# shiinamiyuki/akari_render

Measured on AMD Instinct MI355X. Metric: Msamples/s (whole node), 1080p path tracer, C2, higher is better.
Workload: dtype f32

## Files before the change

akari_render_amd/capi.py:

```python
from __future__ import annotations

import ctypes as C
import os
from typing import Optional

import numpy as np

from . import abi
from .build import LIB, build

AKR_OK = 0
FILM_PLANE_RGB, FILM_PLANE_SPLAT, FILM_PLANE_WEIGHT, FILM_PLANES_PT, FILM_PLANES_ALL = 1, 2, 4, 5, 7
ERR_INVALID_ARGUMENT, ERR_HIP, ERR_NO_DEVICE, ERR_IO, ERR_PARSE, ERR_UNSUPPORTED, ERR_OOM, ERR_RENDER = -1, -2, -3, -4, -5, -6, -7, -8

(ARRAY_WOOP, ARRAY_TRI_GID, ARRAY_SHADE, ARRAY_INSTANCES, ARRAY_MATERIALS, ARRAY_BVH_NODES, ARRAY_LIGHT_ENTRIES,
 ARRAY_LIGHT_PDF, ARRAY_AREA_ENTRIES, ARRAY_AREA_PDF, ARRAY_INST_TRI_OFFSET, ARRAY_R2C, ARRAY_C2W,
 ARRAY_TEX_NODES, ARRAY_TEX_IMAGES, ARRAY_TEX_TEXELS, ARRAY_MAT_INPUTS,
 ARRAY_INST_LEAVES, ARRAY_MESH_TRIS, ARRAY_MESH_POS, ARRAY_MESH_META, ARRAY_MESH_NORMALS,
 ARRAY_ENV_MARGINAL_ENTRIES, ARRAY_ENV_MARGINAL_PDF, ARRAY_ENV_CONDITIONAL_ENTRIES, ARRAY_ENV_CONDITIONAL_PDF, ARRAY_ENV_TEXELS) = range(27)
ENV_LIGHT_INSTANCE = 0xFFFFFFFF

EXPORTS = [
    "akr_last_error", "akr_version", "akr_struct_size", "akr_option_set", "akr_option_get", "akr_context_create",
    "akr_context_destroy", "akr_context_synchronize", "akr_context_device_info", "akr_scene_create", "akr_scene_load",
# ... 6 lines not shown
    "akr_gpt_config_default", "akr_gpt_render", "akr_gpt_begin", "akr_gpt_sample", "akr_gpt_sums", "akr_gpt_sums_read",
    "akr_gpt_sums_write", "akr_gpt_finish", "akr_gpt_abort", "akr_gpt_reduce", "akr_mcmc_config_default", "akr_mcmc_render",
    "akr_film_set_splat_scale", "akr_film_get_splat_scale", "akr_pt_read_sampler_states", "akr_context_device_ordinal",
    "akr_device_count", "akr_comm_unique_id", "akr_comm_create", "akr_comm_wrap", "akr_comm_destroy", "akr_film_reduce",
    "akr_pt_kernel_info", "akr_scene_spec_source", "akr_host_spec_compile", "akr_host_spec_compile_text",
    "akr_film_reduce_planes", "akr_mcmc_render_shard", "akr_mcmc_combine_host", "akr_mcmc_combine",
    "akr_scene_set_environment", "akr_scene_get_environment", "akr_scene_set_lens", "akr_scene_get_lens",
]
TEST_EXPORTS = [
    "akr_probe_material_inputs_host", "akr_host_stdrng_u64", "akr_host_chacha_block", "akr_host_pcg32_states",
    "akr_host_pcg_start", "akr_host_alias_table", "akr_probe_math", "akr_probe_bsdf", "akr_probe_intersect",
    "akr_probe_surface_interaction", "akr_probe_material_inputs", "akr_host_decode_png", "akr_host_decode_jpeg",
    "akr_host_decode_exr", "akr_host_decode_tiff", "akr_host_decode_dds", "akr_host_pmj02bn_tables",
    "akr_probe_material_folded_host", "akr_host_sobol_dim1", "akr_host_fastmod", "akr_host_tri_pretest",
    "akr_probe_env_sample", "akr_probe_env_pdf", "akr_host_lens_ray", "akr_probe_camera_rays",
]


class RenderSession(C.Structure):

    _fields_ = [("save_intermediate", C.c_int32), ("save_stats", C.c_int32), ("name", C.c_char_p),
                ("override_sampler_independent", C.c_int32), ("verbose", C.c_int32)]


class AkariError(RuntimeError):
    def __init__(self, code: int, msg: str):
        super().__init__(f"akari_hip error {code}: {msg}")
        self.code = code


# ... 105 lines not shown
    proto("akr_pt_begin", vp, vp, C.POINTER(abi.PtConfig), vp, vpp)
    proto("akr_pt_passes", vp, u32, i32, up)
    proto("akr_pt_end", vp, C.POINTER(abi.PtStats))
    proto("akr_pt_get_stats", vp, C.POINTER(abi.PtStats))
    proto("akr_render_task", vp, vp, C.c_char_p, C.POINTER(RenderSession), C.POINTER(abi.PtStats))
    proto("akr_image_write", C.c_char_p, fp, u32, u32)
    proto("akr_pt_read_sampler_states", vp, u64p)
    proto("akr_host_stdrng_u64", u64, u32, u64p)
    proto("akr_host_chacha_block", up, u64, u64, i32, up)
    proto("akr_host_pcg32_states", u64, u64, u64p)
    proto("akr_host_pcg_start", u64p, u64)
    proto("akr_host_alias_table", fp, u32, up, fp, fp)
    proto("akr_probe_math", vp, u32, fp, fp, fp, fp)
    proto("akr_probe_bsdf", vp, C.POINTER(abi.MaterialDesc), fp, i32, fp, u32, fp, fp)
    proto("akr_probe_intersect", vp, vp, u32, fp, up, fp)
    proto("akr_probe_surface_interaction", vp, vp, u32, up, fp, fp)
    proto("akr_probe_material_inputs", vp, vp, u32, u32, fp, fp)
    proto("akr_probe_material_inputs_host", vp, u32, u32, u32, fp, fp)
    proto("akr_host_decode_png", C.c_char_p, u64, up, up, C.POINTER(C.c_uint8), u64)
    proto("akr_host_decode_jpeg", C.c_char_p, u64, up, up, C.POINTER(C.c_uint8), u64)
    proto("akr_host_decode_exr", C.c_char_p, u64, up, up, fp, u64)
    proto("akr_host_decode_tiff", C.c_char_p, u64, up, up, C.POINTER(C.c_uint8), u64)
    proto("akr_host_decode_dds", C.c_char_p, u64, up, up, C.POINTER(C.c_uint8), u64)
    proto("akr_host_pmj02bn_tables", up, C.POINTER(C.c_uint16))
    _lib = L
    return L


def check(rc: int) -> None:
    if rc != AKR_OK:
# ... 482 lines not shown
    w = np.ascontiguousarray(weights, dtype=np.float32)
    j = np.zeros(w.size, dtype=np.uint32)
    t = np.zeros(w.size, dtype=np.float32)
    pdf = np.zeros(w.size, dtype=np.float32)
    check(lib().akr_host_alias_table(_fp(w), w.size, _up(j), _fp(t), _fp(pdf)))
    return j, t, pdf


def probe_math(ctx: Context, x: np.ndarray):
    x = np.ascontiguousarray(x, dtype=np.float32)
    s, c, l = (np.zeros_like(x) for _ in range(3))
    check(lib().akr_probe_math(ctx.h, x.size, _fp(x), _fp(s), _fp(c), _fp(l)))
    return s, c, l


def probe_bsdf(ctx: Context, m: abi.MaterialData, mode: int, wo, data: np.ndarray, table: Optional[np.ndarray] = None) -> np.ndarray:
    ms = m.to_struct()
    wo = np.ascontiguousarray(wo, dtype=np.float32)
    data = np.ascontiguousarray(data, dtype=np.float32).reshape(-1, 3)
    out = np.zeros((data.shape[0], 4 if mode == 0 else 8), dtype=np.float32)
    tp = _fp(np.ascontiguousarray(table, dtype=np.float32)) if table is not None else C.POINTER(C.c_float)()
    check(lib().akr_probe_bsdf(ctx.h, C.byref(ms), tp, mode, _fp(wo), data.shape[0], _fp(data), _fp(out)))
    return out


def probe_intersect(ctx: Context, scene: Scene, rays: np.ndarray):
    rays = np.ascontiguousarray(rays, dtype=np.float32).reshape(-1, 8)
    out = np.zeros((rays.shape[0], 3), dtype=np.uint32)
    bary = np.zeros((rays.shape[0], 2), dtype=np.float32)
    check(lib().akr_probe_intersect(ctx.h, scene.h, rays.shape[0], _fp(rays), _up(out), _fp(bary)))
    return out, bary


def probe_surface_interaction(ctx: Context, scene: Scene, inst_prim: np.ndarray, bary: np.ndarray) -> np.ndarray:
    ip = np.ascontiguousarray(inst_prim, dtype=np.uint32).reshape(-1, 2)
    b = np.ascontiguousarray(bary, dtype=np.float32).reshape(-1, 2)
    out = np.zeros((ip.shape[0], 19), dtype=np.float32)
    check(lib().akr_probe_surface_interaction(ctx.h, scene.h, ip.shape[0], _up(ip), _fp(b), _fp(out)))
    return out


def probe_material_inputs(ctx: Optional[Context], scene: Scene, material: int, uv: np.ndarray) -> np.ndarray:
    u = np.ascontiguousarray(uv, dtype=np.float32).reshape(-1, 2)
    out = np.zeros((u.shape[0], 26), dtype=np.float32)
    check(lib().akr_probe_material_inputs(ctx.h if ctx is not None else C.c_void_p(), scene.h, material, u.shape[0], _fp(u), _fp(out)))
    return out
# ... 142 lines not shown
```

akari_render_amd/csrc/device/disect.h:

```cpp
#pragma once
#include "drng.h"
#include "dscene.h"

namespace akr {

template <bool V>
struct BoolTag {
    static constexpr bool value = V;
};

struct Hit {
    float t, u, v;
    uint32_t gid;
};

struct PlaneHit {
    float t, px, py, pz;
};
AKR_HD PlaneHit tri_plane(vec3 o, vec3 d, float4 r2) {
    float dz = __builtin_fmaf(r2.x, d.x, __builtin_fmaf(r2.y, d.y, r2.z * d.z));
    float oz = __builtin_fmaf(r2.x, o.x, __builtin_fmaf(r2.y, o.y, __builtin_fmaf(r2.z, o.z, r2.w)));
    PlaneHit h;
    h.t = div_f(-oz, dz);
    h.px = __builtin_fmaf(h.t, d.x, o.x);
// ... 95 lines not shown
    return best != kInvalid;
}

typedef float v2f __attribute__((ext_vector_type(2)));
typedef float v4f __attribute__((ext_vector_type(4)));
AKR_D float min_raw(float a, float b) {
    float r;
    asm("v_min_f32 %0, %1, %2" : "=v"(r) : "v"(a), "v"(b));
    return r;
}
AKR_D float max_raw(float a, float b) {
    float r;
    asm("v_max_f32 %0, %1, %2" : "=v"(r) : "v"(a), "v"(b));
    return r;
}
template <bool TEX = false>
AKR_D void trace_pair_exhaustive(const DScene& sc, vec3 o, vec3 d, float tmax, uint32_t ex0, vec3 so, vec3 sd, float stmax,
                                 uint32_t sex0, uint32_t sex1, Hit& hit, bool& found, bool& occluded, const float4* lds_recs) {
    float best_t = next_up(tmax);
    uint32_t best = kInvalid;
    float best_u = 0.0f, best_v = 0.0f;
    float occ_margin = -1.0f;
    const uint32_t n = sc.n_tris;
    const v4f* lrec = (const v4f*)lds_recs;
    const bool has_alpha = __builtin_amdgcn_readfirstlane((int)sc.has_alpha) != 0;
    v2f T2 = {0.0f, 0.0f}, hx2 = {0.0f, 0.0f}, hy2 = {0.0f, 0.0f}, hz2 = {0.0f, 0.0f};
    auto record = [&](auto alpha_tag, uint32_t k, const v4f& q0, const v4f& q1, const v4f& q2) {
        constexpr bool ALPHA = decltype(alpha_tag)::value;
        if (!((sc.plane_share_mask >> k) & 1ull)) {
            const PlaneHit a = tri_plane(o, d, make_float4(q2.x, q2.y, q2.z, q2.w)), b = tri_plane(so, sd, make_float4(q2.x, q2.y, q2.z, q2.w));
            T2 = (v2f){a.t, b.t};
            hx2 = (v2f){a.px, b.px}; hy2 = (v2f){a.py, b.py}; hz2 = (v2f){a.pz, b.pz};
        }
        float u, v, su, sv;
        tri_uv(PlaneHit{T2.x, hx2.x, hy2.x, hz2.x}, make_float4(q0.x, q0.y, q0.z, q0.w), make_float4(q1.x, q1.y, q1.z, q1.w), u, v);
        tri_uv(PlaneHit{T2.y, hx2.y, hy2.y, hz2.y}, make_float4(q0.x, q0.y, q0.z, q0.w), make_float4(q1.x, q1.y, q1.z, q1.w), su, sv);
        const v2f u2 = {u, su}, v2 = {v, sv};
        const v2f s2 = {1.0f - (u2.x + v2.x), 1.0f - (u2.y + v2.y)};
        const v2f w2 = {tmax - T2.x, stmax - T2.y};
        float m = min_raw(min_raw(min_raw(u2.x, v2.x), s2.x), min_raw(T2.x, w2.x));
        float sm = min_raw(min_raw(min_raw(u2.y, v2.y), s2.y), min_raw(T2.y, w2.y));
        m = (k == ex0) ? -1.0f : m;
        sm = (k == sex0) ? -1.0f : sm;
        sm = (k == sex1) ? -1.0f : sm;
        if (ALPHA) {
            const uint32_t ka = __builtin_amdgcn_readfirstlane(k);
            if (m >= 0.0f && !alpha_test<TEX>(sc, ka, u2.x, v2.x)) m = -1.0f;
            if (sm >= 0.0f && !alpha_test<TEX>(sc, ka, u2.y, v2.y)) sm = -1.0f;
        }
        const float tc = (m >= 0.0f) ? T2.x : __builtin_inff();
        const bool better = tc < best_t;
        best_t = better ? tc : best_t;
        best = better ? k : best;
        occ_margin = max_raw(occ_margin, sm);
    };
    auto walk = [&](auto alpha_tag) {
        v4f a0 = lrec[0], a1 = lrec[1], a2 = lrec[2], b0, b1, b2;
        uint32_t k = 0;
        for (; k + 1 < n; k += 2) {
            b0 = lrec[3 * (k + 1)]; b1 = lrec[3 * (k + 1) + 1]; b2 = lrec[3 * (k + 1) + 2];
            record(alpha_tag, k, a0, a1, a2);
            a0 = lrec[3 * (k + 2)]; a1 = lrec[3 * (k + 2) + 1]; a2 = lrec[3 * (k + 2) + 2];
            record(alpha_tag, k + 1, b0, b1, b2);
        }
        if (k < n) record(alpha_tag, k, a0, a1, a2);
    };
    if (has_alpha) walk(BoolTag<true>{});
    else walk(BoolTag<false>{});
    if (best != kInvalid) {
        const v4f q0 = lrec[3 * best], q1 = lrec[3 * best + 1];
        const float px = __builtin_fmaf(best_t, d.x, o.x), py = __builtin_fmaf(best_t, d.y, o.y), pz = __builtin_fmaf(best_t, d.z, o.z);
        best_u = __builtin_fmaf(q0.x, px, __builtin_fmaf(q0.y, py, __builtin_fmaf(q0.z, pz, q0.w)));
        best_v = __builtin_fmaf(q1.x, px, __builtin_fmaf(q1.y, py, __builtin_fmaf(q1.z, pz, q1.w)));
    }
    found = best != kInvalid;
    hit.t = found ? best_t : tmax;
    hit.u = best_u;
    hit.v = best_v;
    hit.gid = best;
    occluded = occ_margin >= 0.0f;
}

constexpr uint32_t kBvhDone = 0xfffffffeu;
// ... 235 lines not shown
```

akari_render_amd/csrc/device/dmath.h:

```cpp
#pragma once
#if !defined(__HIPCC_RTC__)
#include <hip/hip_runtime.h>
#include <stdint.h>
#else
typedef unsigned char uint8_t;
typedef unsigned short uint16_t;
typedef int int32_t;
typedef unsigned int uint32_t;
typedef long int64_t;
typedef unsigned long uint64_t;
typedef unsigned long uintptr_t;
typedef unsigned long size_t;
#endif

#define AKR_HD __host__ __device__ __forceinline__
#define AKR_D __device__ __forceinline__

#ifndef AKR_ARITH_RELAXED
#define AKR_ARITH_RELAXED 0
#endif
#if AKR_ARITH_RELAXED && defined(__HIP_DEVICE_COMPILE__)
#define AKR_RX 1
#else
#define AKR_RX 0
// ... 27 lines not shown
AKR_HD vec3 operator-(vec3 a) { return vec3{-a.x, -a.y, -a.z}; }
AKR_HD float dot(vec3 a, vec3 b) { return (a.x * b.x + a.y * b.y) + a.z * b.z; }
AKR_HD vec3 cross(vec3 a, vec3 b) { return vec3{a.y * b.z - a.z * b.y, a.z * b.x - a.x * b.z, a.x * b.y - a.y * b.x}; }
AKR_HD float rcp_f(float x) {
#if AKR_RX && AKR_RX_RCP
    return __builtin_amdgcn_rcpf(x);
#else
    return 1.0f / x;
#endif
}
AKR_HD float div_f(float a, float b) {
#if AKR_RX && AKR_RX_RCP
    return a * __builtin_amdgcn_rcpf(b);
#else
    return a / b;
#endif
}
AKR_HD float sqrt_f(float x) {
#if AKR_RX
    return __builtin_amdgcn_sqrtf(x);
#else
    return __builtin_sqrtf(x);
#endif
}
AKR_HD float length2(vec3 a) { return dot(a, a); }
AKR_HD float length(vec3 a) { return sqrt_f(dot(a, a)); }
AKR_HD vec3 div_s(vec3 a, float s) {
    float inv = rcp_f(s);
    return a * inv;
}
// ... 123 lines not shown
```

akari_render_amd/csrc/device/dscene.h:

```cpp
#pragma once
#include "dtex.h"

namespace akr {

constexpr uint32_t kInvalid = 0xffffffffu;

constexpr uint32_t kBvhNodeWords = 16;
constexpr uint32_t kBvhTriWords = 16;
constexpr uint32_t kBvhStackDepth = 24;

enum : uint32_t { SHADE_ROWS = 8, INST_ROWS = 8 };
enum : uint32_t { TRI_HAS_NORMALS = 1u, TRI_HAS_TANGENTS = 2u };

struct LightRec {
    uint32_t tri_offset, n_tris, first_gid, inst;
};

constexpr uint32_t kMeshPrimMask = 0x7fffffffu, kMeshTriShares = 0x80000000u;
struct DInst {
    const uint4* __restrict__ tlas_leaves;
    const float4* __restrict__ mesh_tris;
    const uint32_t* __restrict__ mesh_pos;
    const uint32_t* __restrict__ mesh_meta;
    const float4* __restrict__ mesh_normals;
// ... 107 lines not shown
```

akari_render_amd/csrc/device/pt_pass.h:

```cpp
#pragma once
#include "dpath.h"

namespace akr {

#ifndef AKR_PT_MIN_WAVES
#define AKR_PT_MIN_WAVES 4
#endif
#ifndef AKR_PT_MIN_WAVES_BVH
#define AKR_PT_MIN_WAVES_BVH 4
#endif
#ifndef AKR_PT_MIN_WAVES_FD
#define AKR_PT_MIN_WAVES_FD 4
#endif
#ifndef AKR_PT_MIN_WAVES_TEX
#define AKR_PT_MIN_WAVES_TEX 3
#endif
#ifndef AKR_PT_MIN_WAVES_BVH_TEX
#define AKR_PT_MIN_WAVES_BVH_TEX 3
#endif
template <bool BVH, bool FD, bool TEX, bool PMJ, bool STAGE, bool DEFER, uint32_t ABSENT = 0, bool INST = false, bool ENV = false, bool LENS = false>
AKR_D void pt_pass_body(const PtParams& p) {
    extern __shared__ __attribute__((aligned(16))) uint32_t lds_stack[];
    TraceCtx tc;
    tc.stack = lds_stack + threadIdx.x;
    tc.cnt = TraceCounters{0, 0, 0};
    PtParams staged = p;
    if (STAGE) stage_scene_tables<BVH, TEX, !BVH && !FD && TEX>(p, lds_stack, staged);
    const PtParams& q = STAGE ? staged : p;
    const DScene& sc = q.sc;
    constexpr bool TILE = BVH && !TEX && !INST;
    constexpr uint32_t STRAG = BVH ? (INST ? AKR_PT_STRAGGLERS_INST : (TEX ? AKR_PT_STRAGGLERS_TEX : AKR_PT_STRAGGLERS)) : 0;
    const uint4* tile = (const uint4*)(lds_stack + p.tile_offset);
    if (TILE) {
        uint32_t* l = lds_stack + p.tile_offset;
// ... 97 lines not shown
                while (phase != 2u) {
                    if (s.active) trav_step<2, TEX, TILE>(sc, s, tc.stack, tc.cnt, phase == 1u, tile);
                    if (!s.active) {
                        if (phase == 0u) {
                            found = s.best != kInvalid;
                            hit.t = s.best_t; hit.u = s.best_u; hit.v = s.best_v; hit.gid = s.best;
                            phase = r.has_shadow ? 1u : 2u;
                            if (r.has_shadow) trav_begin(s, r.s_o, r.s_d, 0.0f, r.s_tmax, r.s_ex0, r.s_ex1);
                        } else {
                            occluded = s.best != kInvalid;
                            phase = 2u;
                        }
                    }
                }
            } else {
                trace_pair_exhaustive<TEX>(sc, r.ro, r.rd, r.has_ray ? 1e20f : -1.0f, r.ray_ex0, r.s_o, r.s_d, r.has_shadow ? r.s_tmax : -1.0f, r.s_ex0, r.s_ex1, hit, found,
                                           occluded, lds_recs);
            }
            if (DEFER) {
                if (r.deferred) {
                    hit.gid = r.d_gid; hit.u = r.d_u; hit.v = r.d_v; hit.t = 0.0f;
                    found = true;
                    r.has_ray = true;
                    r.deferred = false;
                } else if (r.has_ray && found && (iteration & q.defer_metal)) {
                    const uint32_t mat = f2u(sc.shade[(size_t)hit.gid * SHADE_ROWS + 6].y);
                    if (sc.materials[mat].flags & q.defer_flags) {
                        r.d_gid = hit.gid; r.d_u = hit.u; r.d_v = hit.v;
                        r.deferred = true;
                        r.has_ray = false;
                    }
// ... 16 lines not shown
```

akari_render_amd/csrc/host/api_probe.cpp:

```cpp
#if defined(AKR_TEST_HOOKS) && AKR_TEST_HOOKS
#include "api_internal.h"
#include "../../../include/akari_hip_test.h"
#include "../device/dinst.h"
#include "../device/disect.h"
#include "../device/dpath.h"

extern "C" {

AKR_TEST_API int32_t akr_host_stdrng_u64(uint64_t seed, uint32_t n, uint64_t* out) {
    if (!out) return fail(AKR_ERR_INVALID_ARGUMENT, "out is NULL");
    StdRng rng(seed);
    for (uint32_t i = 0; i < n; i++) out[i] = rng.next_u64();
    return AKR_OK;
}
AKR_TEST_API int32_t akr_host_chacha_block(const uint32_t* key8, uint64_t counter, uint64_t stream, int32_t rounds, uint32_t* out16) {
    if (!key8 || !out16) return fail(AKR_ERR_INVALID_ARGUMENT, "NULL argument");
    StdRng::chacha_block(key8, counter, stream, rounds, out16);
    return AKR_OK;
}
AKR_TEST_API int32_t akr_host_pcg32_states(uint64_t seed, uint64_t n, uint64_t* out2n) {
    if (!out2n) return fail(AKR_ERR_INVALID_ARGUMENT, "out is NULL");
    StdRng rng(seed);
    for (uint64_t i = 0; i < n; i++) {
        Pcg32 p = pcg_new_seq_offset(i, rng.next_u64());
// ... 54 lines not shown
    return guarded([&] {
        ctx->bind();
        DevBuf dx, ds, dc, dl;
        std::vector<float> xv(x, x + n);
        dx.upload(xv);
        ds.alloc(n * 4); dc.alloc(n * 4); dl.alloc(n * 4);
        if (n) HIP_CHECK(launch_probe_math(n, dx.as<float>(), ds.as<float>(), dc.as<float>(), dl.as<float>(), ctx->stream));
        HIP_CHECK(hipStreamSynchronize(ctx->stream));
        if (n) {
            HIP_CHECK(hipMemcpy(s, ds.p, n * 4, hipMemcpyDeviceToHost));
            HIP_CHECK(hipMemcpy(c, dc.p, n * 4, hipMemcpyDeviceToHost));
            HIP_CHECK(hipMemcpy(l, dl.p, n * 4, hipMemcpyDeviceToHost));
        }
    });
}
AKR_TEST_API int32_t akr_probe_bsdf(akr_context* ctx, const akr_material_desc* m, const float* table, int32_t mode, const float* wo, uint32_t n,
                               const float* in, float* out) {
    if (!ctx || !m || !wo || !in || !out) return fail(AKR_ERR_INVALID_ARGUMENT, "akr_probe_bsdf: NULL argument");
    return guarded([&] {
        ctx->bind();
        std::vector<DMaterial> dm(1, fold_material(*m));
        DevBuf dmat, dtab, din, dout;
        dmat.upload(dm);
        std::vector<float> tab(4096, 0.0f);
        if (table) tab.assign(table, table + 4096);
        dtab.upload(tab);
        std::vector<float> inv(in, in + 3ull * n);
        din.upload(inv);
        size_t out_n = (mode == 0 ? 4ull : 8ull) * n;
        dout.alloc(out_n * 4);
// ... 11 lines not shown
}
AKR_TEST_API int32_t akr_probe_intersect(akr_context* ctx, akr_scene* scene, uint32_t n, const float* rays, uint32_t* hit_inst_prim, float* bary) {
    if (!ctx || !scene || !rays || !hit_inst_prim || !bary) return fail(AKR_ERR_INVALID_ARGUMENT, "akr_probe_intersect: NULL argument");
    return guarded([&] {
        ctx->bind();
        DevBuf dr, dout, db;
        std::vector<float> rv(rays, rays + 8ull * n);
        dr.upload(rv);
        dout.alloc(3ull * n * 4);
        db.alloc(2ull * n * 4);
        if (n) HIP_CHECK(launch_probe_intersect(probe_params(scene), n, dr.as<float>(), dout.as<uint32_t>(), db.as<float>(), ctx->stream));
        HIP_CHECK(hipStreamSynchronize(ctx->stream));
        if (n) {
            HIP_CHECK(hipMemcpy(hit_inst_prim, dout.p, 3ull * n * 4, hipMemcpyDeviceToHost));
            HIP_CHECK(hipMemcpy(bary, db.p, 2ull * n * 4, hipMemcpyDeviceToHost));
        }
    });
}
static int32_t probe_env(akr_context* ctx, akr_scene* scene, uint32_t mode, uint32_t n, const float* in, float* out, const char* name) {
    if (!ctx || !scene || !in || !out) return fail(AKR_ERR_INVALID_ARGUMENT, std::string(name) + ": NULL argument");
    if (scene->ctx != ctx || !scene->cs.env.on) return fail(AKR_ERR_INVALID_ARGUMENT, std::string(name) + ": the scene has no environment light on this context");
    return guarded([&] {
        ctx->bind();
        const size_t n_in = (mode == 0 ? 2ull : 3ull) * n, n_out = (mode == 0 ? 5ull : 4ull) * n;
        DevBuf din, dout;
        din.upload(std::vector<float>(in, in + n_in));
        dout.alloc(n_out * 4);
        if (n) HIP_CHECK(launch_probe_env(probe_params(scene), mode, n, din.as<float>(), dout.as<float>(), ctx->stream));
        HIP_CHECK(hipStreamSynchronize(ctx->stream));
        if (n) HIP_CHECK(hipMemcpy(out, dout.p, n_out * 4, hipMemcpyDeviceToHost));
// ... 212 lines not shown
```

akari_render_amd/csrc/host/api_scene.cpp:

```cpp
#include "api_internal.h"

static void ensure_ggx_table(akr_scene* s) {
    akr_context* ctx = s->ctx;
    if (!s->flat.ggx_table.empty()) {
        s->ggx_host = s->flat.ggx_table;
    } else if (s->cs.needs_ggx_table) {
        std::lock_guard<std::mutex> lock(ctx->ggx_mutex);
        if (!ctx->ggx_cache.empty()) {
            s->ggx_host = ctx->ggx_cache;
            s->ggx_table.upload(s->ggx_host);
            return;
        }
        std::vector<uint64_t> seeds(4096);
        StdRng rng(0);
        for (auto& v : seeds) v = rng.next_u64();
        DevBuf dseeds;
        dseeds.upload(seeds);
        s->ggx_table.alloc(4096 * sizeof(float));
        HIP_CHECK(launch_ggx_table(dseeds.as<uint64_t>(), s->ggx_table.as<float>(), 1u << 20, ctx->stream));
        HIP_CHECK(hipStreamSynchronize(ctx->stream));
        s->ggx_host.resize(4096);
        HIP_CHECK(hipMemcpy(s->ggx_host.data(), s->ggx_table.p, 4096 * sizeof(float), hipMemcpyDeviceToHost));
        ctx->ggx_cache = s->ggx_host;
        return;
// ... 69 lines not shown
    d.area_alias = s->area_alias.as<AliasPacked>();
    d.lights = s->lights.as<LightRec>();
    d.n_lights = cs.n_lights;
    d.env = cs.env.on ? s->env_rec.as<DEnv>() : nullptr;
}
static void count_device_bytes(akr_scene* s) {
    s->device_bytes = 0;
    for (const DevBuf* b : {&s->woop, &s->tri_gid, &s->shade, &s->normals, &s->inst, &s->materials, &s->ggx_table, &s->light_entries,
                            &s->light_pdf, &s->light_inst, &s->light_tri_offset, &s->light_n_tris, &s->area_entries, &s->area_pdf,
                            &s->inst_tri_offset, &s->light_alias, &s->area_alias, &s->lights, &s->bvh_nodes, &s->tex_nodes, &s->tex_images, &s->tex_texels, &s->tex_mat_inputs,
                            &s->in2_tlas_leaves, &s->in2_mesh_tris, &s->in2_mesh_pos, &s->in2_mesh_meta, &s->in2_mesh_normals, &s->in2_inst_mats, &s->in2_share_bits,
                            &s->env_texels, &s->env_marginal, &s->env_conditional, &s->env_rec})
        s->device_bytes += b->bytes;
}

static void check_lens_reach(const akr_scene* s, const HostLens& lens) {
    const CompiledScene& cs = s->cs;
    if (lens.radius == 0.0f || (cs.bvh_nodes.empty() && !cs.instanced.on)) return;
    const float* c2w = s->flat.camera.c2w;
    float bound[3], moved[16];
    lens_origin_bound(c2w, lens.radius, bound);
    std::memcpy(moved, c2w, sizeof moved);
    bool inside = true;
    for (int a = 0; a < 3; a++) {
        const float m = std::max(std::max(std::fabs(cs.scene_lo[a]), std::fabs(cs.scene_hi[a])), std::fabs(c2w[12 + a]));
        if (bound[a] > m) inside = false;
        moved[12 + a] = bound[a];
    }
    if (inside || (!cs.instanced.on && bvh_box_padding(cs.scene_lo, cs.scene_hi, moved) == bvh_box_padding(cs.scene_lo, cs.scene_hi, c2w))) return;
    char msg[320];
// ... 3 lines not shown
}

void akr_api::scene_finish(akr_scene* s) {
    akr_context* ctx = s->ctx;
    compile_scene(s->flat, s->cs);
    compile_environment(s->flat, s->cs);
    check_lens_reach(s, s->flat.lens);
    CompiledScene& cs = s->cs;
    camera_matrices(s->flat.camera, s->r2c, s->c2w, &s->c2w_identity);
    if (!ctx) {
        s->ggx_host = s->flat.ggx_table.empty() ? std::vector<float>(4096, 0.0f) : s->flat.ggx_table;
        std::memset(&s->dscene, 0, sizeof s->dscene);
        return;
    }
    ctx->bind();
    s->woop.upload(cs.woop);
    s->tri_gid.upload(cs.tri_gid);
    s->shade.upload(cs.shade);
    s->normals.upload(cs.normals);
    s->inst.upload(cs.inst);
    s->materials.upload(cs.materials);
    s->area_entries.upload(cs.area_entries);
    s->area_pdf.upload(cs.area_pdf);
    s->inst_tri_offset.upload(cs.inst_tri_offset);
    s->bvh_nodes.upload(cs.instanced.on ? cs.instanced.nodes : cs.bvh_nodes);
    if (cs.instanced.on) {
        s->in2_tlas_leaves.upload(cs.instanced.tlas_leaves);
        s->in2_mesh_tris.upload(cs.instanced.mesh_tris);
        s->in2_mesh_pos.upload(cs.instanced.mesh_pos);
        s->in2_mesh_meta.upload(cs.instanced.mesh_meta);
// ... 355 lines not shown
```

akari_render_amd/csrc/kernels.h:

```cpp
#pragma once
#if !defined(__HIPCC_RTC__)
#include <hip/hip_runtime.h>
#endif

#include "device/drng.h"
#include "device/dscene.h"

namespace akr {

#ifndef AKR_PT_STRAGGLERS
#define AKR_PT_STRAGGLERS 8
#endif
#ifndef AKR_PT_STRAGGLERS_TEX
#define AKR_PT_STRAGGLERS_TEX 0
#endif
#ifndef AKR_PT_STRAGGLERS_INST
#define AKR_PT_STRAGGLERS_INST 8
#endif
constexpr uint32_t kParkSlots = 16, kParkSlotsNoDefer = 13;
constexpr uint32_t kCarrySlots = 13;
constexpr uint32_t kCarrySlotsInstanced = 16;
constexpr size_t kBlueNoiseColumnBytes = 48 * 256 * 2;
struct PtLdsPlan {
    size_t recs_bytes, park_bytes, carry_bytes;
// ... 154 lines not shown
hipError_t launch_aov(const PtParams& p, uint32_t spp, uint32_t aov, uint32_t remap, hipStream_t stream);
hipError_t launch_wf_init(const PtParams& p, const WfBuffers& wf, hipStream_t stream);
hipError_t launch_wf_shade(const PtParams& p, const WfBuffers& wf, uint32_t q_out, hipStream_t stream);
hipError_t launch_wf_shade_env(const PtParams& p, const WfBuffers& wf, uint32_t q_out, hipStream_t stream);
uint32_t wf_trace_blocks_per_cu(const PtParams& p);
hipError_t launch_wf_trace(const PtParams& p, const WfBuffers& wf, uint32_t q_in, uint32_t n_blocks, hipStream_t stream);
size_t wf_sort_temp_bytes(uint32_t n);
hipError_t wf_sort_pairs(void* temp, size_t temp_bytes, const uint32_t* keys_in, uint32_t* keys_out, const uint32_t* vals_in, uint32_t* vals_out, uint32_t n, hipStream_t stream);
hipError_t launch_probe_material(const PtParams& p, uint32_t material, uint32_t n, const float* uv, uint32_t* out, hipStream_t stream);
hipError_t launch_init_pcg32(const uint64_t* seeds, void* states, uint64_t n, hipStream_t stream);
hipError_t launch_film_resolve(const float* film, uint64_t n, float splat_scale, float* rgb, hipStream_t stream);
hipError_t launch_ggx_table(const uint64_t* seeds, float* table, uint32_t samples, hipStream_t stream);
hipError_t launch_probe_math(uint32_t n, const float* x, float* s, float* c, float* l, hipStream_t stream);
hipError_t launch_probe_bsdf(const DMaterial* m, const float* table, int mode, const float* wo, uint32_t n, const float* in, float* out,
                             hipStream_t stream);
hipError_t launch_probe_intersect(const PtParams& p, uint32_t n, const float* rays, uint32_t* out, float* bary, hipStream_t stream);
hipError_t launch_probe_si(const PtParams& p, uint32_t n, const uint32_t* inst_prim, const float* bary, float* out, hipStream_t stream);
#endif

}
```

akari_render_amd/csrc/pt_kernels.hip:

```cpp
#include <algorithm>
#include "device/pt_pass.h"
#include "pt_launch.h"

namespace akr {

__global__ void k_init_pcg32(const uint64_t* __restrict__ seeds, Pcg32* __restrict__ states, uint64_t n) {
    uint64_t i = (uint64_t)blockIdx.x * blockDim.x + threadIdx.x;
    if (i < n) states[i] = pcg_new_seq_offset(i, seeds[i]);
}

__global__ void k_film_resolve(const float* __restrict__ film, uint64_t n, float splat_scale, float* __restrict__ rgb) {
    uint64_t i = (uint64_t)blockIdx.x * blockDim.x + threadIdx.x;
    if (i >= n) return;
    float w = film[6 * n + i];
    float inv = w == 0.0f ? 1.0f : w;
#pragma unroll
    for (int c = 0; c < 3; c++) rgb[3 * i + c] = film[3 * i + c] / inv + film[3 * n + 3 * i + c] * splat_scale;
}

__global__ void k_ggx_dielectric_table(const uint64_t* __restrict__ seeds, float* __restrict__ table, uint32_t samples) {
    const uint32_t dim = 16;
    uint32_t gid = blockIdx.x * blockDim.x + threadIdx.x;
    if (gid >= dim * dim * dim) return;
    uint32_t tx = gid % dim, ty = (gid / dim) % dim, tz = gid / (dim * dim);
// ... 23 lines not shown
        }
        sum += val;
    }
    table[gid] = sum / (float)samples;
}

__global__ void k_probe_math(uint32_t n, const float* __restrict__ x, float* s, float* c, float* l) {
    uint32_t i = blockIdx.x * blockDim.x + threadIdx.x;
    if (i >= n) return;
    float sv, cv;
    sincos_f(x[i], sv, cv);
    s[i] = sv;
    c[i] = cv;
    l[i] = log_f(x[i]);
}
__global__ void k_probe_bsdf(const DMaterial* __restrict__ m, const float* __restrict__ table, int mode, vec3 wo, uint32_t n,
                             const float* __restrict__ in, float* __restrict__ out) {
    uint32_t i = blockIdx.x * blockDim.x + threadIdx.x;
    if (i >= n) return;
    ShadePoint sp;
    shade_point_init(sp, *m, frame_from_n(mk3(0, 0, 1)), mk3(0, 0, 1), false);
    if (mode == 0) {
        BsdfEval e = shade_evaluate(sp, *m, table, wo, mk3(in[3 * i], in[3 * i + 1], in[3 * i + 2]));
        out[4 * i + 0] = e.f.x;
        out[4 * i + 1] = e.f.y;
        out[4 * i + 2] = e.f.z;
        out[4 * i + 3] = e.pdf;
    } else {
        BsdfSample s = shade_sample(sp, *m, table, wo, in[3 * i], mk2(in[3 * i + 1], in[3 * i + 2]));
        float* o = out + 8 * (size_t)i;
// ... 15 lines not shown
    Hit h;
    bool found = INST ? trace_inst<false, false>(p.sc, mk3(r[0], r[1], r[2]), mk3(r[3], r[4], r[5]), r[6], r[7], kInvalid, kInvalid, h, tc.stack, tc.cnt)
                      : trace<BVH, false>(p, tc, mk3(r[0], r[1], r[2]), mk3(r[3], r[4], r[5]), r[6], r[7], kInvalid, kInvalid, h);
    if (!act) return;
    uint32_t inst = 0, prim = 0;
    if (found) {
        inst = INST ? inst_of_gid(p.sc, h.gid) : f2u(p.sc.shade[(size_t)h.gid * SHADE_ROWS + 6].z);
        prim = h.gid - p.sc.inst_tri_offset[inst];
    }
    out[3 * i + 0] = found ? 1u : 0u;
    out[3 * i + 1] = inst;
    out[3 * i + 2] = prim;
    bary[2 * i + 0] = found ? h.u : 0.0f;
    bary[2 * i + 1] = found ? h.v : 0.0f;
}
template <bool INST>
__global__ void k_probe_si(PtParams p, uint32_t n, const uint32_t* __restrict__ inst_prim, const float* __restrict__ bary, float* __restrict__ out) {
    uint32_t i = blockIdx.x * blockDim.x + threadIdx.x;
    if (i >= n) return;
    uint32_t gid = p.sc.inst_tri_offset[inst_prim[2 * i]] + inst_prim[2 * i + 1];
    SurfacePoint s = surface_interaction_any<INST>(p.sc, gid, mk2(bary[2 * i], bary[2 * i + 1]));
    float* o = out + 19 * (size_t)i;
    o[0] = s.p.x; o[1] = s.p.y; o[2] = s.p.z;
    o[3] = s.ng.x; o[4] = s.ng.y; o[5] = s.ng.z;
    o[6] = s.frame.n.x; o[7] = s.frame.n.y; o[8] = s.frame.n.z;
    o[9] = s.frame.t.x; o[10] = s.frame.t.y; o[11] = s.frame.t.z;
    o[12] = s.frame.s.x; o[13] = s.frame.s.y; o[14] = s.frame.s.z;
    o[15] = s.uv.x;
    o[16] = s.uv.y;
    o[17] = s.prim_area;
// ... 32 lines not shown
}
hipError_t launch_film_resolve(const float* film, uint64_t n, float splat_scale, float* rgb, hipStream_t stream) {
    uint32_t blocks = (uint32_t)((n + 255) / 256);
    if (blocks == 0) return hipSuccess;
    hipLaunchKernelGGL(k_film_resolve, dim3(blocks), dim3(256), 0, stream, film, n, splat_scale, rgb);
    return hipGetLastError();
}
hipError_t launch_ggx_table(const uint64_t* seeds, float* table, uint32_t samples, hipStream_t stream) {
    hipLaunchKernelGGL(k_ggx_dielectric_table, dim3(64), dim3(64), 0, stream, seeds, table, samples);
    return hipGetLastError();
}
hipError_t launch_probe_math(uint32_t n, const float* x, float* s, float* c, float* l, hipStream_t stream) {
    hipLaunchKernelGGL(k_probe_math, dim3((n + 255) / 256), dim3(256), 0, stream, n, x, s, c, l);
    return hipGetLastError();
}
hipError_t launch_probe_bsdf(const DMaterial* m, const float* table, int mode, const float* wo, uint32_t n, const float* in, float* out,
                             hipStream_t stream) {
    hipLaunchKernelGGL(k_probe_bsdf, dim3((n + 255) / 256), dim3(256), 0, stream, m, table, mode, mk3(wo[0], wo[1], wo[2]), n, in, out);
    return hipGetLastError();
}
hipError_t launch_probe_intersect(const PtParams& p, uint32_t n, const float* rays, uint32_t* out, float* bary, hipStream_t stream) {
    const bool bvh = p.sc.bvh_nodes != nullptr, inst = p.sc.in2.on != 0;
    dispatch_bools([&](auto B, auto I) {
        launch_kernel(k_probe_intersect<B() || I(), I()>, (n + 255) / 256, B() || I() ? p.sc.bvh_stack_depth * 256 * 4 : 0, stream, p, n, rays, out, bary);
    }, bvh, inst);
    return hipGetLastError();
}
hipError_t launch_probe_si(const PtParams& p, uint32_t n, const uint32_t* inst_prim, const float* bary, float* out, hipStream_t stream) {
    dispatch_bools([&](auto I) { launch_kernel(k_probe_si<I()>, (n + 255) / 256, 0, stream, p, n, inst_prim, bary, out); }, p.sc.in2.on != 0);
    return hipGetLastError();
// ... 4 lines not shown
```

Before: 3166.

## Use unscaled Newton division in exhaustive pair walk with wave-uniform IEEE fallback

Replaces the scaled IEEE division in the per-triangle plane test of the small-scene exhaustive pair walk with an rcp plus Newton-refinement division that skips denormal scaling. A host-computed origin bound is stored in the woop array. Waves whose rays exceed that bound, or whose plane distances get too small, redo the walk with the exact IEEE path. This cuts the division cost in the hot untextured trace loop, but adds the bound check, a ballot and a possible full redo for the whole wave. Probe kernels are added to test the new division and the pair walk.

```diff
diff --git a/akari_render_amd/capi.py b/akari_render_amd/capi.py
--- a/akari_render_amd/capi.py
+++ b/akari_render_amd/capi.py
@@ -44,6 +44,7 @@
     "akr_host_decode_exr", "akr_host_decode_tiff", "akr_host_decode_dds", "akr_host_pmj02bn_tables",
     "akr_probe_material_folded_host", "akr_host_sobol_dim1", "akr_host_fastmod", "akr_host_tri_pretest",
     "akr_probe_env_sample", "akr_probe_env_pdf", "akr_host_lens_ray", "akr_probe_camera_rays",
+    "akr_probe_div", "akr_probe_intersect_pair",
 ]
 
 
@@ -179,6 +180,8 @@
     proto("akr_probe_math", vp, u32, fp, fp, fp, fp)
     proto("akr_probe_bsdf", vp, C.POINTER(abi.MaterialDesc), fp, i32, fp, u32, fp, fp)
     proto("akr_probe_intersect", vp, vp, u32, fp, up, fp)
+    proto("akr_probe_div", vp, u32, fp, fp, fp, fp)
+    proto("akr_probe_intersect_pair", vp, vp, u32, fp, up, up, fp)
     proto("akr_probe_surface_interaction", vp, vp, u32, up, fp, fp)
     proto("akr_probe_material_inputs", vp, vp, u32, u32, fp, fp)
     proto("akr_probe_material_inputs_host", vp, u32, u32, u32, fp, fp)
@@ -691,6 +694,15 @@
     return s, c, l
 
 
+def probe_div(ctx: Context, a: np.ndarray, b: np.ndarray):
+    a = np.ascontiguousarray(a, dtype=np.float32)
+    b = np.ascontiguousarray(b, dtype=np.float32)
+    assert a.shape == b.shape
+    fast, ieee = np.zeros_like(a), np.zeros_like(a)
+    check(lib().akr_probe_div(ctx.h, a.size, _fp(a), _fp(b), _fp(fast), _fp(ieee)))
+    return fast, ieee
+
+
 def probe_bsdf(ctx: Context, m: abi.MaterialData, mode: int, wo, data: np.ndarray, table: Optional[np.ndarray] = None) -> np.ndarray:
     ms = m.to_struct()
     wo = np.ascontiguousarray(wo, dtype=np.float32)
@@ -707,6 +719,16 @@
     bary = np.zeros((rays.shape[0], 2), dtype=np.float32)
     check(lib().akr_probe_intersect(ctx.h, scene.h, rays.shape[0], _fp(rays), _up(out), _fp(bary)))
     return out, bary
+
+
+def probe_intersect_pair(ctx: Context, scene: Scene, rays: np.ndarray, excl: np.ndarray):
+    rays = np.ascontiguousarray(rays, dtype=np.float32).reshape(-1, 16)
+    excl = np.ascontiguousarray(excl, dtype=np.uint32).reshape(-1, 3)
+    assert rays.shape[0] == excl.shape[0]
+    out = np.zeros((rays.shape[0], 4), dtype=np.uint32)
+    tuv = np.zeros((rays.shape[0], 3), dtype=np.float32)
+    check(lib().akr_probe_intersect_pair(ctx.h, scene.h, rays.shape[0], _fp(rays), _up(excl), _up(out), _fp(tuv)))
+    return out, tuv
 
 
 def probe_surface_interaction(ctx: Context, scene: Scene, inst_prim: np.ndarray, bary: np.ndarray) -> np.ndarray:
diff --git a/akari_render_amd/csrc/device/disect.h b/akari_render_amd/csrc/device/disect.h
--- a/akari_render_amd/csrc/device/disect.h
+++ b/akari_render_amd/csrc/device/disect.h
@@ -133,9 +133,41 @@
     asm("v_max_f32 %0, %1, %2" : "=v"(r) : "v"(a), "v"(b));
     return r;
 }
-template <bool TEX = false>
+AKR_D float min_abs_raw(float a, float b) {
+    float r;
+    asm("v_min_f32 %0, %1, |%2|" : "=v"(r) : "v"(a), "v"(b));
+    return r;
+}
+AKR_D float max3_abs_raw(float a, float b, float c) {
+    float r;
+    asm("v_max3_f32 %0, |%1|, |%2|, |%3|" : "=v"(r) : "v"(a), "v"(b), "v"(c));
+    return r;
+}
+AKR_D PlaneHit tri_plane_unscaled(vec3 o, vec3 d, float4 r2, float& lo) {
+    float dz = __builtin_fmaf(r2.x, d.x, __builtin_fmaf(r2.y, d.y, r2.z * d.z));
+    float oz = __builtin_fmaf(r2.x, o.x, __builtin_fmaf(r2.y, o.y, __builtin_fmaf(r2.z, o.z, r2.w)));
+    lo = min_abs_raw(lo, oz);
+    PlaneHit h;
+    h.t = div_f_unscaled(-oz, dz);
+    h.px = __builtin_fmaf(h.t, d.x, o.x);
+    h.py = __builtin_fmaf(h.t, d.y, o.y);
+    h.pz = __builtin_fmaf(h.t, d.z, o.z);
+    return h;
+}
+
+template <bool DIV>
+struct WalkOpt {
+    static constexpr bool unscaled_div = DIV;
+};
+template <int V>
+struct IntTag {
+    static constexpr int value = V;
+};
+
+template <bool TEX = false, class OPT = WalkOpt<true>>
 AKR_D void trace_pair_exhaustive(const DScene& sc, vec3 o, vec3 d, float tmax, uint32_t ex0, vec3 so, vec3 sd, float stmax,
-                                 uint32_t sex0, uint32_t sex1, Hit& hit, bool& found, bool& occluded, const float4* lds_recs) {
+                                 uint32_t sex0, uint32_t sex1, Hit& hit, bool& found, bool& occluded, const float4* lds_recs, uint32_t* took_ieee_walk = nullptr) {
+    constexpr bool UNSCALED = OPT::unscaled_div && !AKR_RX;
     float best_t = next_up(tmax);
     uint32_t best = kInvalid;
     float best_u = 0.0f, best_v = 0.0f;
@@ -144,10 +176,13 @@
     const v4f* lrec = (const v4f*)lds_recs;
     const bool has_alpha = __builtin_amdgcn_readfirstlane((int)sc.has_alpha) != 0;
     v2f T2 = {0.0f, 0.0f}, hx2 = {0.0f, 0.0f}, hy2 = {0.0f, 0.0f}, hz2 = {0.0f, 0.0f};
-    auto record = [&](auto alpha_tag, uint32_t k, const v4f& q0, const v4f& q1, const v4f& q2) {
-        constexpr bool ALPHA = decltype(alpha_tag)::value;
+    float lo = __builtin_inff(), slo = __builtin_inff();
+    auto record = [&](auto alpha_tag, auto div_tag, uint32_t k, const v4f& q0, const v4f& q1, const v4f& q2) {
+        constexpr int ALPHA = decltype(alpha_tag)::value;
+        constexpr bool FAST = decltype(div_tag)::value;
         if (!((sc.plane_share_mask >> k) & 1ull)) {
-            const PlaneHit a = tri_plane(o, d, make_float4(q2.x, q2.y, q2.z, q2.w)), b = tri_plane(so, sd, make_float4(q2.x, q2.y, q2.z, q2.w));
+            const float4 r2 = make_float4(q2.x, q2.y, q2.z, q2.w);
+            const PlaneHit a = FAST ? tri_plane_unscaled(o, d, r2, lo) : tri_plane(o, d, r2), b = FAST ? tri_plane_unscaled(so, sd, r2, slo) : tri_plane(so, sd, r2);
             T2 = (v2f){a.t, b.t};
             hx2 = (v2f){a.px, b.px}; hy2 = (v2f){a.py, b.py}; hz2 = (v2f){a.pz, b.pz};
         }
@@ -162,7 +197,7 @@
         m = (k == ex0) ? -1.0f : m;
         sm = (k == sex0) ? -1.0f : sm;
         sm = (k == sex1) ? -1.0f : sm;
-        if (ALPHA) {
+        if (ALPHA == 1 || (ALPHA == 2 && has_alpha)) {
             const uint32_t ka = __builtin_amdgcn_readfirstlane(k);
             if (m >= 0.0f && !alpha_test<TEX>(sc, ka, u2.x, v2.x)) m = -1.0f;
             if (sm >= 0.0f && !alpha_test<TEX>(sc, ka, u2.y, v2.y)) sm = -1.0f;
@@ -174,18 +209,42 @@
         occ_margin = max_raw(occ_margin, sm);
     };
     auto walk = [&](auto alpha_tag) {
+        const BoolTag<UNSCALED> div_tag{};
         v4f a0 = lrec[0], a1 = lrec[1], a2 = lrec[2], b0, b1, b2;
         uint32_t k = 0;
         for (; k + 1 < n; k += 2) {
             b0 = lrec[3 * (k + 1)]; b1 = lrec[3 * (k + 1) + 1]; b2 = lrec[3 * (k + 1) + 2];
-            record(alpha_tag, k, a0, a1, a2);
+            record(alpha_tag, div_tag, k, a0, a1, a2);
             a0 = lrec[3 * (k + 2)]; a1 = lrec[3 * (k + 2) + 1]; a2 = lrec[3 * (k + 2) + 2];
-            record(alpha_tag, k + 1, b0, b1, b2);
-        }
-        if (k < n) record(alpha_tag, k, a0, a1, a2);
+            record(alpha_tag, div_tag, k + 1, b0, b1, b2);
+        }
+        if (k < n) record(alpha_tag, div_tag, k, a0, a1, a2);
     };
-    if (has_alpha) walk(BoolTag<true>{});
-    else walk(BoolTag<false>{});
+    auto walk_ieee = [&] {
+        best_t = next_up(tmax); best = kInvalid; occ_margin = -1.0f;
+#pragma clang loop unroll(disable)
+        for (uint32_t k = 0; k < n; k++) {
+            record(IntTag<2>{}, BoolTag<false>{}, k, lrec[3 * k], lrec[3 * k + 1], lrec[3 * k + 2]);
+        }
+    };
+    if (UNSCALED) {
+        const float ob = lds_recs[3u * (n + 1u) + 2u].w;
+        const bool pre_bad = ((tmax >= 0.0f) & !((max3_abs_raw(o.x, o.y, o.z) <= ob) & (max3_abs_raw(d.x, d.y, d.z) <= 2.0f) & (tmax <= 1e20f))) |
+                             ((stmax >= 0.0f) & !((max3_abs_raw(so.x, so.y, so.z) <= ob) & (max3_abs_raw(sd.x, sd.y, sd.z) <= 2.0f) & (stmax <= 1e20f)));
+        bool redo = __builtin_amdgcn_ballot_w64(pre_bad) != 0;
+        if (!redo) {
+            if (has_alpha) walk(IntTag<1>{});
+            else walk(IntTag<0>{});
+            const bool bad = ((tmax >= 0.0f) & (lo < 0x1p-47f)) | ((stmax >= 0.0f) & (slo < 0x1p-47f));
+            redo = __builtin_amdgcn_ballot_w64(bad) != 0;
+        }
+        if (redo) walk_ieee();
+        if (took_ieee_walk) *took_ieee_walk = redo ? 1u : 0u;
+    } else {
+        if (has_alpha) walk(IntTag<1>{});
+        else walk(IntTag<0>{});
+        if (took_ieee_walk) *took_ieee_walk = 0u;
+    }
     if (best != kInvalid) {
         const v4f q0 = lrec[3 * best], q1 = lrec[3 * best + 1];
         const float px = __builtin_fmaf(best_t, d.x, o.x), py = __builtin_fmaf(best_t, d.y, o.y), pz = __builtin_fmaf(best_t, d.z, o.z);
diff --git a/akari_render_amd/csrc/device/dmath.h b/akari_render_amd/csrc/device/dmath.h
--- a/akari_render_amd/csrc/device/dmath.h
+++ b/akari_render_amd/csrc/device/dmath.h
@@ -65,6 +65,20 @@
     return a * __builtin_amdgcn_rcpf(b);
 #else
     return a / b;
+#endif
+}
+AKR_HD float div_f_unscaled(float a, float b) {
+#if defined(__HIP_DEVICE_COMPILE__) && !AKR_RX
+    const float r0 = __builtin_amdgcn_rcpf(b);
+    const float e0 = __builtin_fmaf(-b, r0, 1.0f);
+    const float r1 = __builtin_fmaf(e0, r0, r0);
+    const float q0 = a * r1;
+    const float e1 = __builtin_fmaf(-b, q0, a);
+    const float q1 = __builtin_fmaf(e1, r1, q0);
+    const float e2 = __builtin_fmaf(-b, q1, a);
+    return __builtin_fmaf(e2, r1, q1);
+#else
+    return div_f(a, b);
 #endif
 }
 AKR_HD float sqrt_f(float x) {
diff --git a/akari_render_amd/csrc/device/dscene.h b/akari_render_amd/csrc/device/dscene.h
--- a/akari_render_amd/csrc/device/dscene.h
+++ b/akari_render_amd/csrc/device/dscene.h
@@ -8,6 +8,7 @@
 constexpr uint32_t kBvhNodeWords = 16;
 constexpr uint32_t kBvhTriWords = 16;
 constexpr uint32_t kBvhStackDepth = 24;
+AKR_HD uint32_t walk_bound_word(uint32_t n_tris) { return 12u * (n_tris + 1u) + 11u; }
 
 enum : uint32_t { SHADE_ROWS = 8, INST_ROWS = 8 };
 enum : uint32_t { TRI_HAS_NORMALS = 1u, TRI_HAS_TANGENTS = 2u };
diff --git a/akari_render_amd/csrc/device/pt_pass.h b/akari_render_amd/csrc/device/pt_pass.h
--- a/akari_render_amd/csrc/device/pt_pass.h
+++ b/akari_render_amd/csrc/device/pt_pass.h
@@ -18,6 +18,8 @@
 #ifndef AKR_PT_MIN_WAVES_BVH_TEX
 #define AKR_PT_MIN_WAVES_BVH_TEX 3
 #endif
+template <bool TEX>
+using PairWalkOpt = WalkOpt<!TEX>;
 template <bool BVH, bool FD, bool TEX, bool PMJ, bool STAGE, bool DEFER, uint32_t ABSENT = 0, bool INST = false, bool ENV = false, bool LENS = false>
 AKR_D void pt_pass_body(const PtParams& p) {
     extern __shared__ __attribute__((aligned(16))) uint32_t lds_stack[];
@@ -145,7 +147,7 @@
                     }
                 }
             } else {
-                trace_pair_exhaustive<TEX>(sc, r.ro, r.rd, r.has_ray ? 1e20f : -1.0f, r.ray_ex0, r.s_o, r.s_d, r.has_shadow ? r.s_tmax : -1.0f, r.s_ex0, r.s_ex1, hit, found,
+                trace_pair_exhaustive<TEX, PairWalkOpt<TEX>>(sc, r.ro, r.rd, r.has_ray ? 1e20f : -1.0f, r.ray_ex0, r.s_o, r.s_d, r.has_shadow ? r.s_tmax : -1.0f, r.s_ex0, r.s_ex1, hit, found,
                                            occluded, lds_recs);
             }
             if (DEFER) {
diff --git a/akari_render_amd/csrc/host/api_probe.cpp b/akari_render_amd/csrc/host/api_probe.cpp
--- a/akari_render_amd/csrc/host/api_probe.cpp
+++ b/akari_render_amd/csrc/host/api_probe.cpp
@@ -92,6 +92,22 @@
         }
     });
 }
+AKR_TEST_API int32_t akr_probe_div(akr_context* ctx, uint32_t n, const float* a, const float* b, float* out_fast, float* out_ieee) {
+    if (!ctx || !a || !b || !out_fast || !out_ieee) return fail(AKR_ERR_INVALID_ARGUMENT, "akr_probe_div: NULL argument");
+    return guarded([&] {
+        ctx->bind();
+        DevBuf da, db, df, di;
+        da.upload(std::vector<float>(a, a + n));
+        db.upload(std::vector<float>(b, b + n));
+        df.alloc((size_t)n * 4); di.alloc((size_t)n * 4);
+        if (n) HIP_CHECK(launch_probe_div(n, da.as<float>(), db.as<float>(), df.as<float>(), di.as<float>(), ctx->stream));
+        HIP_CHECK(hipStreamSynchronize(ctx->stream));
+        if (n) {
+            HIP_CHECK(hipMemcpy(out_fast, df.p, (size_t)n * 4, hipMemcpyDeviceToHost));
+            HIP_CHECK(hipMemcpy(out_ieee, di.p, (size_t)n * 4, hipMemcpyDeviceToHost));
+        }
+    });
+}
 AKR_TEST_API int32_t akr_probe_bsdf(akr_context* ctx, const akr_material_desc* m, const float* table, int32_t mode, const float* wo, uint32_t n,
                                const float* in, float* out) {
     if (!ctx || !m || !wo || !in || !out) return fail(AKR_ERR_INVALID_ARGUMENT, "akr_probe_bsdf: NULL argument");
@@ -133,6 +149,26 @@
         if (n) {
             HIP_CHECK(hipMemcpy(hit_inst_prim, dout.p, 3ull * n * 4, hipMemcpyDeviceToHost));
             HIP_CHECK(hipMemcpy(bary, db.p, 2ull * n * 4, hipMemcpyDeviceToHost));
+        }
+    });
+}
+AKR_TEST_API int32_t akr_probe_intersect_pair(akr_context* ctx, akr_scene* scene, uint32_t n, const float* rays16, const uint32_t* excl3, uint32_t* out4, float* tuv3) {
+    if (!ctx || !scene || !rays16 || !excl3 || !out4 || !tuv3) return fail(AKR_ERR_INVALID_ARGUMENT, "akr_probe_intersect_pair: NULL argument");
+    if (scene->ctx != ctx) return fail(AKR_ERR_INVALID_ARGUMENT, "akr_probe_intersect_pair: scene belongs to another context");
+    if (scene->dscene.bvh_nodes || scene->dscene.in2.on || scene->dscene.n_tris > 64)
+        return fail(AKR_ERR_INVALID_ARGUMENT, "akr_probe_intersect_pair: the pair walk serves scenes of at most 64 triangles");
+    return guarded([&] {
+        ctx->bind();
+        DevBuf dr, de, dout, dt;
+        dr.upload(std::vector<float>(rays16, rays16 + 16ull * n));
+        de.upload(std::vector<uint32_t>(excl3, excl3 + 3ull * n));
+        dout.alloc(4ull * n * 4);
+        dt.alloc(3ull * n * 4);
+        if (n) HIP_CHECK(launch_probe_intersect_pair(probe_params(scene), n, dr.as<float>(), de.as<uint32_t>(), dout.as<uint32_t>(), dt.as<float>(), ctx->stream));
+        HIP_CHECK(hipStreamSynchronize(ctx->stream));
+        if (n) {
+            HIP_CHECK(hipMemcpy(out4, dout.p, 4ull * n * 4, hipMemcpyDeviceToHost));
+            HIP_CHECK(hipMemcpy(tuv3, dt.p, 3ull * n * 4, hipMemcpyDeviceToHost));
         }
     });
 }
diff --git a/akari_render_amd/csrc/host/api_scene.cpp b/akari_render_amd/csrc/host/api_scene.cpp
--- a/akari_render_amd/csrc/host/api_scene.cpp
+++ b/akari_render_amd/csrc/host/api_scene.cpp
@@ -107,6 +107,21 @@
         s->device_bytes += b->bytes;
 }
 
+static float walk_origin_bound(const std::vector<float>& woop, uint32_t n) {
+    double s_max = 0.0, w_max = 0.0;
+    for (uint32_t k = 0; k < n; k++) {
+        const float* r = &woop[12ull * k + 8];
+        if (!(std::isfinite(r[0]) && std::isfinite(r[1]) && std::isfinite(r[2]) && std::isfinite(r[3]))) return -1.0f;
+        s_max = std::max(s_max, std::fabs((double)r[0]) + std::fabs((double)r[1]) + std::fabs((double)r[2]));
+        w_max = std::max(w_max, std::fabs((double)r[3]));
+    }
+    const double limit = 0x1p45;
+    if (!(2.0 * s_max <= limit && w_max < limit)) return -1.0f;
+    double b = 0x1p40;
+    while (b >= 0x1p-40 && s_max * b + w_max > limit) b *= 0.5;
+    return b >= 0x1p-40 ? (float)b : -1.0f;
+}
+
 static void check_lens_reach(const akr_scene* s, const HostLens& lens) {
     const CompiledScene& cs = s->cs;
     if (lens.radius == 0.0f || (cs.bvh_nodes.empty() && !cs.instanced.on)) return;
@@ -140,6 +155,8 @@
         return;
     }
     ctx->bind();
+    if (cs.bvh_nodes.empty() && !cs.instanced.on && cs.woop.size() > walk_bound_word(cs.n_tris))
+        cs.woop[walk_bound_word(cs.n_tris)] = walk_origin_bound(cs.woop, cs.n_tris);
     s->woop.upload(cs.woop);
     s->tri_gid.upload(cs.tri_gid);
     s->shade.upload(cs.shade);
diff --git a/akari_render_amd/csrc/kernels.h b/akari_render_amd/csrc/kernels.h
--- a/akari_render_amd/csrc/kernels.h
+++ b/akari_render_amd/csrc/kernels.h
@@ -192,6 +192,8 @@
 hipError_t launch_probe_math(uint32_t n, const float* x, float* s, float* c, float* l, hipStream_t stream);
 hipError_t launch_probe_bsdf(const DMaterial* m, const float* table, int mode, const float* wo, uint32_t n, const float* in, float* out,
                              hipStream_t stream);
+hipError_t launch_probe_div(uint32_t n, const float* a, const float* b, float* out_fast, float* out_ieee, hipStream_t stream);
+hipError_t launch_probe_intersect_pair(const PtParams& p, uint32_t n, const float* rays, const uint32_t* excl, uint32_t* out, float* out_tuv, hipStream_t stream);
 hipError_t launch_probe_intersect(const PtParams& p, uint32_t n, const float* rays, uint32_t* out, float* bary, hipStream_t stream);
 hipError_t launch_probe_si(const PtParams& p, uint32_t n, const uint32_t* inst_prim, const float* bary, float* out, hipStream_t stream);
 #endif
diff --git a/akari_render_amd/csrc/pt_kernels.hip b/akari_render_amd/csrc/pt_kernels.hip
--- a/akari_render_amd/csrc/pt_kernels.hip
+++ b/akari_render_amd/csrc/pt_kernels.hip
@@ -61,6 +61,12 @@
     c[i] = cv;
     l[i] = log_f(x[i]);
 }
+__global__ void k_probe_div(uint32_t n, const float* __restrict__ a, const float* __restrict__ b, float* __restrict__ out_fast, float* __restrict__ out_ieee) {
+    uint32_t i = blockIdx.x * blockDim.x + threadIdx.x;
+    if (i >= n) return;
+    out_fast[i] = div_f_unscaled(a[i], b[i]);
+    out_ieee[i] = div_f(a[i], b[i]);
+}
 __global__ void k_probe_bsdf(const DMaterial* __restrict__ m, const float* __restrict__ table, int mode, vec3 wo, uint32_t n,
                              const float* __restrict__ in, float* __restrict__ out) {
     uint32_t i = blockIdx.x * blockDim.x + threadIdx.x;
@@ -106,6 +112,30 @@
     bary[2 * i + 0] = found ? h.u : 0.0f;
     bary[2 * i + 1] = found ? h.v : 0.0f;
 }
+__global__ __launch_bounds__(256) void k_probe_intersect_pair(PtParams p, uint32_t n, const float* __restrict__ rays, const uint32_t* __restrict__ excl, uint32_t* __restrict__ out,
+                                                              float* __restrict__ out_tuv) {
+    extern __shared__ __attribute__((aligned(16))) uint32_t lds_stack[];
+    const uint32_t* g = (const uint32_t*)p.sc.woop;
+    for (uint32_t i = threadIdx.x; i < (p.sc.n_tris + 2u) * 12u; i += 256u) lds_stack[i] = g[i];
+    __syncthreads();
+    const uint32_t i = blockIdx.x * blockDim.x + threadIdx.x;
+    const bool act = i < n;
+    const float* r = rays + 16 * (size_t)(act ? i : 0);
+    const uint32_t* e = excl + 3 * (size_t)(act ? i : 0);
+    Hit h;
+    bool found = false, occluded = false;
+    uint32_t redo = 0;
+    trace_pair_exhaustive<false>(p.sc, mk3(r[0], r[1], r[2]), mk3(r[3], r[4], r[5]), act ? r[6] : -1.0f, e[0], mk3(r[8], r[9], r[10]), mk3(r[11], r[12], r[13]),
+                                 act ? r[14] : -1.0f, e[1], e[2], h, found, occluded, (const float4*)lds_stack, &redo);
+    if (!act) return;
+    out[4 * i + 0] = found ? 1u : 0u;
+    out[4 * i + 1] = h.gid;
+    out[4 * i + 2] = occluded ? 1u : 0u;
+    out[4 * i + 3] = redo;
+    out_tuv[3 * i + 0] = h.t;
+    out_tuv[3 * i + 1] = h.u;
+    out_tuv[3 * i + 2] = h.v;
+}
 template <bool INST>
 __global__ void k_probe_si(PtParams p, uint32_t n, const uint32_t* __restrict__ inst_prim, const float* __restrict__ bary, float* __restrict__ out) {
     uint32_t i = blockIdx.x * blockDim.x + threadIdx.x;
@@ -168,6 +198,14 @@
     hipLaunchKernelGGL(k_probe_math, dim3((n + 255) / 256), dim3(256), 0, stream, n, x, s, c, l);
     return hipGetLastError();
 }
+hipError_t launch_probe_div(uint32_t n, const float* a, const float* b, float* out_fast, float* out_ieee, hipStream_t stream) {
+    hipLaunchKernelGGL(k_probe_div, dim3((n + 255) / 256), dim3(256), 0, stream, n, a, b, out_fast, out_ieee);
+    return hipGetLastError();
+}
+hipError_t launch_probe_intersect_pair(const PtParams& p, uint32_t n, const float* rays, const uint32_t* excl, uint32_t* out, float* out_tuv, hipStream_t stream) {
+    launch_kernel(k_probe_intersect_pair, (n + 255) / 256, (p.sc.n_tris + 2u) * 48u, stream, p, n, rays, excl, out, out_tuv);
+    return hipGetLastError();
+}
 hipError_t launch_probe_bsdf(const DMaterial* m, const float* table, int mode, const float* wo, uint32_t n, const float* in, float* out,
                              hipStream_t stream) {
     hipLaunchKernelGGL(k_probe_bsdf, dim3((n + 255) / 256), dim3(256), 0, stream, m, table, mode, mk3(wo[0], wo[1], wo[2]), n, in, out);
```

Result: faster. 3249 (median of 6 runs) (+2.6%).
